# Stanford-ILIAD/Diverse-Conventions

Measured on NVIDIA B200. Metric: agent-steps/sec (env+obs), higher is better.
Workload: dtype u8

## Files before the change

### diverse_conventions_b200/csrc/policy_kernels.cu

```cuda
#include <cuda_bf16.h>
#include <cuda_runtime.h>
#include <stdint.h>
#include <stdlib.h>
#include <string.h>

#include <new>
#include <vector>

#include "api_common.h"
#include "oc_core.cuh"
#include "oc_device.cuh"
#include "mixed_schedule.h"
#include "ocb.h"
#include "policy_internal.h"

using namespace ocb;

namespace {

constexpr int kRows = 128;
constexpr int kHid = 64;
constexpr int kCo = 32;
constexpr int kSlots = 16;
constexpr int kK1 = 9 * kSlots;
// ... 406 lines not shown
    PB_COL_EMPTY = B_COL_EMPTY,
    PB_D1_FULL = 8,
    PB_A2_FULL = 10,
    PB_A2_EMPTY = 12,
    PB_D2_FULL = 14,
    PB_D3_FULL = 16,
    PB_D3_EMPTY = 18,
    PB_HEAD_FULL = 20,
    PB_HEAD_EMPTY = 21,
    PB_W_FULL = 24,
    PB_W_EMPTY = 48,
    PB_D1_EMPTY = 72,
    PBS_D1_FULL = 74,
    PBS_D1_EMPTY = 78,
    PB_COUNT = 82,
    PB_TMEM_SLOT = 120
};

struct PairSmemLayout {
    int stage, head, wring, bars, total;
};
__host__ __device__ inline PairSmemLayout pair_smem_layout(int npos, int ring, int stage_stride) {
    PairSmemLayout s;
    const BlobLayout L = blob_layout(npos);
    int o = 0;
    s.stage = o, o += al128(kLoadWarps * 32 * stage_stride * 4);
    s.head = o, o += kPRestOff + 2 * (L.head_bytes - L.bias1);
    s.wring = o, o += ring * kChunk;
    s.bars = o, o += 1024;
    s.total = o + 128;
    return s;
}

template <bool kProf, bool kPop = false, bool kMix = false>
__device__ __forceinline__ void pair_producer_role(long long* pw, const PolicyParams& prm, int t0, int t1, const BlobLayout L,
                                                   uint32_t s_head, uint32_t s_wring, uint32_t bars,
                                                   const uint8_t* mix_partner = nullptr) {
    const int nets = prm.single ? 1 : 2;
    const int R = prm.pair_ring, nch = nets * L.chunks;
    const bool resident = R >= nch;
    const bool static_w = resident && prm.tile_policy == nullptr;
    const int Reff = resident ? nch : R;
    const uint32_t rest = (uint32_t)(L.head_bytes - L.bias1);
    uint32_t u = 0, round = 0;
    int slot = 0;
    for (int t = t0; t < t1; ++t, ++u) {
        if (static_w && u > 0) break;
        const bool chg = blob_changed(prm, t, t0);
        const int tp = tile_pol(prm, t);
        const bool cross = prm.f_vt_round != 0 && prm.tile_policy != nullptr;
        const uint8_t* blob_a = prm.blobs + ((size_t)(cross ? (tp & 0xFFFF) : tp) * 2 + (prm.single == 2 ? 1 : 0)) * prm.blob_stride;
        const uint8_t* blob_c = kMix ? mix_partner
                                     : cross && !kPop ? prm.blobs + (size_t)(tp >> 16) * 2 * prm.blob_stride : blob_a + prm.blob_stride;
        if (chg) {
            if (u > 0) mbar_wait_p<kProf>(bars + 8 * (PB_HEAD_EMPTY + ((u - 1) & 1)), ((u - 1) >> 1) & 1, pw[PW_HEAD_EMPTY]);
            if (elect_one()) {
                const uint32_t hb = bars + 8 * PB_HEAD_FULL;
                mbar_arrive_expect_tx(hb, (uint32_t)nets * (2u * kPConvBytes + rest));
                bulk_g2s(s_head, blob_a + L.wc_hi, kPConvBytes, hb);
                bulk_g2s(s_head + 2 * kPConvBytes, blob_a + L.wc_lo, kPConvBytes, hb);
                bulk_g2s(s_head + kPRestOff, blob_a + L.bias1, rest, hb);
                if (nets == 2) {
                    bulk_g2s(s_head + kPConvBytes, blob_c + L.wc_hi, kPConvBytes, hb);
                    bulk_g2s(s_head + 3 * kPConvBytes, blob_c + L.wc_lo, kPConvBytes, hb);
                    bulk_g2s(s_head + kPRestOff + rest, blob_c + L.bias1, rest, hb);
                }
            }
            __syncwarp();
        }
        const bool load = !resident || chg;
        for (int j = 0; j < L.chunks; ++j) {
#pragma unroll
            for (int g = 0; g < 2; ++g) {
                if (g >= nets) break;
                if (round > 0) mbar_wait_p<kProf>(bars + 8 * (PB_W_EMPTY + slot), (round - 1) & 1, pw[PW_W_EMPTY]);
                if (load) {
                    if (elect_one()) {
                        mbar_arrive_expect_tx(bars + 8 * (PB_W_FULL + slot), kChunk);
                        bulk_g2s(s_wring + slot * kChunk, (g ? blob_c : blob_a) + L.head_bytes + (size_t)j * kChunk, kChunk,
                                 bars + 8 * (PB_W_FULL + slot));
                    }
                    __syncwarp();
                }
                if (++slot == Reff) slot = 0, ++round;
            }
        }
    }
}

template <bool kProf, int kNet>
__device__ __forceinline__ void pair_conv_role(long long* pw, const PolicyParams& prm, int t0, int t1, const BlobLayout L, uint32_t tmem,
                                               uint32_t a_head, uint32_t bars, const int cp0 = 0, const int cpstep = 1,
                                               const uint32_t ring = kColRing, const int col_full = PB_COL_FULL,
                                               const int col_empty = PB_COL_EMPTY) {
    const int W = prm.W, H = prm.H, PH = H - 2, npos = prm.npos;
    constexpr int kN = kNet < 0 ? kHid : kCo;
    const uint32_t idesc = make_idesc(kRows, kN);
    const uint32_t a_wchi = a_head + (kNet == 1 ? kPConvBytes : 0), a_wclo = a_wchi + 2 * kPConvBytes;
    const int b_full = kNet < 0 ? PB_D1_FULL : PBS_D1_FULL + 2 * kNet, b_empty = kNet < 0 ? PB_D1_EMPTY : PBS_D1_EMPTY + 2 * kNet;
    uint32_t head_gen = 0, u = 0;
    uint32_t uses[2] = {0, 0};
    const bool tracer = kNet <= 0;
    uint32_t t_slot = 0, t_round = 0;
    auto advance = [&](uint32_t& slot, uint32_t& round, int n) {
        for (int i = 0; i < n; ++i)
            if (++slot == ring) slot = 0, ++round;
    };

    for (int t = t0; t < t1; ++t, ++u) {
        if (blob_changed(prm, t, t0)) {
            mbar_wait_p<kProf>(bars + 8 * PB_HEAD_FULL, head_gen & 1, pw[PW_HEAD_FULL]);
            ++head_gen;
        }
        if (kNet == 1) {
            const int s_last = (npos - 1) & 1;
            const uint32_t cum = (u + 1) * (uint32_t)((npos + 1 - s_last) / 2);
            mbar_wait_p<kProf>(bars + 8 * (PBS_D1_FULL + s_last), (cum - 1) & 1, pw[PW_D3_FULL]);
        }
        uint32_t w_slot = t_slot, w_round = t_round;
        uint32_t r_slot = t_slot;
        uint32_t c_slot = t_slot;
        int cols_seen = 0, released = 0, ox = 0, oy = cp0;
        while (oy >= PH) oy -= PH, ++ox, c_slot = (c_slot + 1 == ring) ? 0 : c_slot + 1;
        for (int cp = cp0; cp < npos; cp += cpstep) {
            const int st = cp & 1;
            for (; cols_seen < ox + 3; ++cols_seen) {
                mbar_wait_p<kProf>(bars + 8 * (col_full + w_slot), w_round & 1, pw[PW_COL_FULL]);
                if (++w_slot == ring) w_slot = 0, ++w_round;
            }
            if (uses[st] > 0) mbar_wait_p<kProf>(bars + 8 * (b_empty + st), (uses[st] - 1) & 1, pw[PW_D1_FULL]);
            if (u > 0 && cp < 2 && !prm.single)
                mbar_wait_p<kProf>(bars + 8 * (PB_D3_EMPTY + (kNet < 0 ? cp : kNet)), (u - 1) & 1, pw[PW_D3_FULL]);
            tc_fence_after();
            const uint32_t d1 = tmem + kPColD1 + (kNet < 0 ? st * kHid : kNet * kHid + st * kCo);
            int nox = ox, noy = oy + cpstep;
            uint32_t n_slot = c_slot;
            while (noy >= PH) noy -= PH, ++nox, n_slot = (n_slot + 1 == ring) ? 0 : n_slot + 1;
            const int keep = cp + cpstep < npos ? nox : W;
            const uint32_t s1 = (c_slot + 1 >= ring) ? c_slot + 1 - ring : c_slot + 1;
            const uint32_t s2 = (c_slot + 2 >= ring) ? c_slot + 2 - ring : c_slot + 2;
            const uint32_t cellb = tmem + kColCells + (uint32_t)oy * kCellCols, colw = (uint32_t)H * kCellCols;
            const uint32_t cb0 = cellb + c_slot * colw, cb1 = cellb + s1 * colw, cb2 = cellb + s2 * colw;
            const long long ti0 = kProf ? clock64() : 0;
            if (cp == 3 && tracer) trace_ev<kProf>(prm, t - t0, 54);
            if (cp < 2 && tracer) trace_ev<kProf>(prm, t - t0, 11 + cp);
            if (elect_one()) {
#pragma unroll
                for (int j = 0; j < 9; ++j) {
                    const int dx = j / 3, dy = j - dx * 3;
                    const uint32_t ta = (dx == 0 ? cb0 : dx == 1 ? cb1 : cb2) + dy * kCellCols;
                    umma_bf16_ts(d1, ta, make_desc(a_wchi + j * 256, 128, 2304), idesc, j > 0);
                    umma_bf16_ts(d1, ta, make_desc(a_wclo + j * 256, 128, 2304), idesc, 1);
                }
                umma_commit(bars + 8 * (b_full + st));
                uint32_t rs = r_slot;
                for (int c = released; c < keep; ++c) {
                    umma_commit(bars + 8 * (col_empty + rs));
                    rs = (rs + 1 == ring) ? 0 : rs + 1;
                }
                if (cp + cpstep >= npos) umma_commit(bars + 8 * (PB_HEAD_EMPTY + (u & 1)));
            }
            __syncwarp();
            for (; released < keep; ++released) r_slot = (r_slot + 1 == ring) ? 0 : r_slot + 1;
            if (kProf) pw[PW_ISSUE_CONV] += clock64() - ti0;
            if (cp < 8 && tracer) trace_ev<kProf>(prm, t - t0, 16 + cp);
            ++uses[st];
            ox = nox, oy = noy, c_slot = n_slot;
        }
        advance(t_slot, t_round, W);
    }
}

template <bool kProf, bool kSplit>
__device__ __forceinline__ void pair_fc_role(long long* pw, const PolicyParams& prm, const int g, int t0, int t1, const BlobLayout L,
                                             uint32_t tmem, uint32_t a_wring, uint32_t bars) {
    const int npos = prm.npos;
    const int nets = prm.single ? 1 : 2;
    const int R = prm.pair_ring, nch = nets * L.chunks;
    const bool resident = R >= nch;
    const bool static_w = resident && prm.tile_policy == nullptr;
    const int Reff = resident ? nch : R;
    const uint32_t idesc = make_idesc(kRows, kHid);
    const uint32_t a_hi = tmem + kPColA2 + g * kA2Cols, a_lo = a_hi + 16;
    uint32_t item = 0, u = 0, w_gen = 0, wround = 0;
    int slot = g;
// ... 106 lines not shown
#pragma unroll 1
        for (int half = 0; half < 2; ++half) {
            float v[32];
            tmem_ld32(trow + kPColD2 + g * kHid + half * 32, v);
            publish(v, s_b1 + half * 32);
        }

        const uint32_t drawn = net == 0 ? out.draw(t, trow_id) : 0u;
        mbar_wait_p<kProf>(bars + 8 * (PB_D3_FULL + g), u & 1, pw[PW_D3_FULL]);
        if (kProf && (warp & 3) == 0) trace_ev<kProf>(prm, trace_vt, g == 0 ? 49 : 52);
        tc_fence_after();
        float head[6];
#pragma unroll
        for (int a = 0; a < 6; ++a) head[a] = s_bh[a];
#pragma unroll 1
        for (int half = 0; half < 2; ++half) {
            float v[32];
            tmem_ld32(trow + kPColD1 + g * kHid + half * 32, v);
            if (half == 1) {
                tc_fence_before();
                mbar_arrive(bars + 8 * (PB_D3_EMPTY + g));
            }
            head_accumulate(net, v, s_b2 + half * 32, s_wh, half * 32, head);
        }
        mbar_arrive(bars + 8 * (PB_HEAD_EMPTY + (u & 1)));
        if (kProf && (warp & 3) == 0) trace_ev<kProf>(prm, trace_vt, g == 0 ? 50 : 53);
        out(t, trow_id, net, head, drawn);
        if (kProf && warp == 0) trace_ev<kProf>(prm, trace_vt, 51);
    }
}
constexpr int kSColD3 = kPColD2 + kHid;
constexpr int kSHeadGroup = 1;

template <bool kProf>
__device__ __forceinline__ void single_fc_role(long long* pw, const PolicyParams& prm, int t0, int t1, const BlobLayout L, uint32_t tmem,
                                               uint32_t a_wring, uint32_t bars) {
    const int npos = prm.npos;
    const int R = prm.pair_ring, nch = L.chunks;
    const bool resident = R >= nch;
    const bool static_w = resident && prm.tile_policy == nullptr;
    const int Reff = resident ? nch : R;
    const uint32_t idesc = make_idesc(kRows, kHid);
    uint32_t u = 0, w_gen = 0, wround = 0;
    uint32_t cnt0 = 0, cnt1 = 0;
    int slot = 0;
    for (int t = t0; t < t1; ++t, ++u) {
        const bool chg = blob_changed(prm, t, t0);
        const bool w_loaded = !resident || chg;
        if (resident && w_loaded) ++w_gen;
        for (int j = 0; j < npos + 2; ++j) {
            const int sg = j < npos ? (j & 1) : (j - npos);
            const uint32_t k = sg ? cnt1 : cnt0;
            mbar_wait_p<kProf>(bars + 8 * (PB_A2_FULL + sg), k & 1, pw[PW_A2_FULL]);
            if (sg) ++cnt1; else ++cnt0;
            if (j == npos && u > 0) mbar_wait_p<kProf>(bars + 8 * PB_D3_EMPTY, (u - 1) & 1, pw[PW_D3_FULL]);
            if (w_loaded) mbar_wait_p<kProf>(bars + 8 * (PB_W_FULL + slot), resident ? ((w_gen - 1) & 1) : (wround & 1), pw[PW_W_FULL]);
            tc_fence_after();
            const uint32_t dst = tmem + (j < npos ? kPColD2 : kSColD3);
            const bool first = (j == 0 || j == npos);
            const uint32_t a_hi = tmem + kPColA2 + sg * kA2Cols, a_lo = a_hi + 16;
            const uint32_t b_hi = a_wring + slot * kChunk, b_lo = b_hi + 4096;
            const long long tf0 = kProf ? clock64() : 0;
            if (elect_one()) {
#pragma unroll
                for (int ks = 0; ks < 2; ++ks) {
                    const uint64_t bhi = make_desc(b_hi + ks * 256, 128, 512), blo = make_desc(b_lo + ks * 256, 128, 512);
                    umma_bf16_ts(dst, a_hi + ks * 8, bhi, idesc, (!first || ks != 0) ? 1u : 0u);
                    umma_bf16_ts(dst, a_hi + ks * 8, blo, idesc, 1);
                    umma_bf16_ts(dst, a_lo + ks * 8, bhi, idesc, 1);
                }
                umma_commit(bars + 8 * (PB_A2_EMPTY + sg));
                if (!static_w) umma_commit(bars + 8 * (PB_W_EMPTY + slot));
                if (j == npos - 1) umma_commit(bars + 8 * PB_D2_FULL);
                if (j == npos + 1) umma_commit(bars + 8 * PB_D3_FULL);
            }
            __syncwarp();
            if (kProf) pw[PW_ISSUE_FC] += clock64() - tf0;
            if (++slot >= Reff) slot = 0, ++wround;
        }
    }
}

template <bool kProf, class Out>
__device__ __forceinline__ void single_epilogue_role(long long* pw, const PolicyParams& prm, int t0, int t1, const BlobLayout L,
                                                     uint32_t tmem, const uint8_t* s_head, uint32_t bars, Out&& out) {
    const int warp = threadIdx.x >> 5, g = warp >> 2, trow_id = (warp & 3) * 32 + (threadIdx.x & 31);
    const int npos = prm.npos;
    const int net = prm.single == 2 ? 1 : 0;
    const uint32_t trow = tmem + ((uint32_t)((warp & 3) * 32) << 16);
    const uint8_t* rest = s_head + kPRestOff - L.bias1;
    const float* s_bias1 = reinterpret_cast<const float*>(rest + L.bias1);
    const float* s_b1 = reinterpret_cast<const float*>(rest + L.b1);
    const float* s_b2 = reinterpret_cast<const float*>(rest + L.b2);
    const float* s_wh = reinterpret_cast<const float*>(rest + L.wh);
    const float* s_bh = reinterpret_cast<const float*>(rest + L.bh);
    uint32_t u = 0, head_gen = 0, pubs = 0, d1_uses = 0;
    auto publish = [&](float (&v)[32], const float* bias) {
        const uint32_t a2 = trow + kPColA2 + g * kA2Cols;
        const float4* b4 = reinterpret_cast<const float4*>(bias);
        uint32_t hi[16], lo[16];
#pragma unroll
        for (int q = 0; q < 8; ++q) {
            const float4 b = b4[q];
            split2(fmaxf(v[4 * q] + b.x, 0.0f), fmaxf(v[4 * q + 1] + b.y, 0.0f), hi[2 * q], lo[2 * q]);
            split2(fmaxf(v[4 * q + 2] + b.z, 0.0f), fmaxf(v[4 * q + 3] + b.w, 0.0f), hi[2 * q + 1], lo[2 * q + 1]);
        }
        if (pubs >= 1) {
            mbar_wait_p<kProf>(bars + 8 * (PB_A2_EMPTY + g), (pubs - 1) & 1, pw[PW_A2_EMPTY]);
            tc_fence_after();
        }
        tmem_st16(a2, hi);
        tmem_st16(a2 + 16, lo);
        tmem_st_wait();
        tc_fence_before();
        mbar_arrive(bars + 8 * (PB_A2_FULL + g));
        ++pubs;
    };
    for (int t = t0; t < t1; ++t, ++u) {
        if (blob_changed(prm, t, t0)) {
            mbar_wait_p<kProf>(bars + 8 * PB_HEAD_FULL, head_gen & 1, pw[PW_HEAD_FULL]);
            ++head_gen;
        }
        for (int j = g; j < npos; j += 2, ++d1_uses) {
            mbar_wait_p<kProf>(bars + 8 * (PBS_D1_FULL + g), d1_uses & 1, pw[PW_D1_FULL]);
            tc_fence_after();
            float v[32];
            tmem_ld32(trow + kPColD1 + g * kCo, v);
            tc_fence_before();
            mbar_arrive(bars + 8 * (PBS_D1_EMPTY + g));
            publish(v, s_bias1 + j * kCo);
        }
        mbar_wait_p<kProf>(bars + 8 * PB_D2_FULL, u & 1, pw[PW_D2_FULL]);
        tc_fence_after();
        {
            float v[32];
            tmem_ld32(trow + kPColD2 + g * 32, v);
            publish(v, s_b1 + g * 32);
        }
        if (g != kSHeadGroup) {
            mbar_arrive(bars + 8 * (PB_HEAD_EMPTY + (u & 1)));
            continue;
        }
        const uint32_t drawn = net == 0 ? out.draw(t, trow_id) : 0u;
        mbar_wait_p<kProf>(bars + 8 * PB_D3_FULL, u & 1, pw[PW_D3_FULL]);
        tc_fence_after();
        float head[6];
#pragma unroll
        for (int a = 0; a < 6; ++a) head[a] = s_bh[a];
#pragma unroll 1
        for (int half = 0; half < 2; ++half) {
            float v[32];
            tmem_ld32(trow + kSColD3 + half * 32, v);
            if (half == 1) {
                tc_fence_before();
                mbar_arrive(bars + 8 * PB_D3_EMPTY);
            }
            head_accumulate(net, v, s_b2 + half * 32, s_wh, half * 32, head);
        }
        mbar_arrive(bars + 8 * (PB_HEAD_EMPTY + (u & 1)));
        out(t, trow_id, net, head, drawn);
    }
}

struct PairForwardOut {
    const PolicyParams& prm;
    unsigned long long offset;
    __device__ __forceinline__ PairForwardOut(const PolicyParams& p) : prm(p), offset(p.offset) {
        if (p.d_offset != nullptr) offset += *p.d_offset;
    }
    __device__ __forceinline__ uint32_t draw(int t, int trow_id) const {
        if (prm.deterministic || prm.given_actions != nullptr || !(prm.actions || prm.logp)) return 0u;
        return policy_draw(prm, (uint32_t)((long long)t * kRows + trow_id), offset);
    }
    __device__ __forceinline__ void operator()(int t, int trow_id, int net, const float (&head)[6], uint32_t drawn) const {
        const long long row = (long long)t * kRows + trow_id;
        if (row < prm.M) {
            if (net == 1) {
                if (prm.values) prm.values[row] = head[0];
            } else {
                emit_actor_row(prm, row, (uint32_t)row, head, offset, false, &drawn);
            }
        }
    }
};

template <bool kProf>
__global__ void __launch_bounds__(kPThreads, 1) policy_pair_kernel(const PolicyParams prm) {
    extern __shared__ uint8_t smem_raw[];
    uint8_t* smem = smem_raw + ((128u - (smem_addr(smem_raw) & 127u)) & 127u);
    const int tid = threadIdx.x, warp = tid >> 5;
// ... 199 lines not shown
        }
        p->pair_ring = ring;
        p->pair_smem_bytes = (size_t)pair_smem_layout(p->npos, ring, p->stage_stride).total;
    } else if (c5_smem_layout(p->npos, p->stage_stride).total > kSmemBudget + 128) {
        delete p;
        return fail(OCB_ERR_UNSUPPORTED, "layout too large for the hidden-512 conv kernel (%d x %d)", cfg->width, cfg->height);
    }
    DeviceGuard guard(device);
    const size_t bytes = generic ? 256 : (size_t)n_policies * 2 * (hidden == kHid ? (size_t)p->L.total : p->L5.total);
    cudaError_t err = cudaDeviceGetAttribute(&p->sm_count, cudaDevAttrMultiProcessorCount, device);
    if (err == cudaSuccess) err = cudaMalloc(&p->d_blobs, bytes);
    if (err == cudaSuccess) err = cudaMemset(p->d_blobs, 0, bytes);
    if (generic) {
        const size_t gbytes = (size_t)n_policies * 2 * p->LG.total * sizeof(float);
        if (err == cudaSuccess) err = cudaMalloc(&p->d_gblobs, gbytes);
        if (err == cudaSuccess) err = cudaMemset(p->d_gblobs, 0, gbytes);
        if (err == cudaSuccess) err = cudaFuncSetAttribute(policy_generic_kernel<kHid>, cudaFuncAttributeMaxDynamicSharedMemorySize, kSmemBudget + 128);
        if (err == cudaSuccess) err = cudaFuncSetAttribute(policy_generic_kernel<kH5>, cudaFuncAttributeMaxDynamicSharedMemorySize, kSmemBudget + 128);
    }
    const int smem_max = kSmemBudget + 128;
    if (err == cudaSuccess) err = cudaFuncSetAttribute(policy_pair_kernel<false>, cudaFuncAttributeMaxDynamicSharedMemorySize, smem_max);
    if (err == cudaSuccess) err = cudaFuncSetAttribute(policy_pair_kernel<true>, cudaFuncAttributeMaxDynamicSharedMemorySize, smem_max);
    if (err == cudaSuccess) err = cudaFuncSetAttribute(rollout_fused_kernel<false, false, 1>, cudaFuncAttributeMaxDynamicSharedMemorySize, smem_max);
    if (err == cudaSuccess) err = cudaFuncSetAttribute(rollout_fused_kernel<true, false, 1>, cudaFuncAttributeMaxDynamicSharedMemorySize, smem_max);
    if (err == cudaSuccess) err = cudaFuncSetAttribute(rollout_fused_kernel<false, true, 1>, cudaFuncAttributeMaxDynamicSharedMemorySize, smem_max);
    if (err == cudaSuccess) err = cudaFuncSetAttribute(rollout_fused_kernel<true, true, 1>, cudaFuncAttributeMaxDynamicSharedMemorySize, smem_max);
    if (err == cudaSuccess) err = cudaFuncSetAttribute(rollout_fused_kernel<false, false, 2>, cudaFuncAttributeMaxDynamicSharedMemorySize, smem_max);
    if (err == cudaSuccess) err = cudaFuncSetAttribute(rollout_fused_kernel<true, false, 2>, cudaFuncAttributeMaxDynamicSharedMemorySize, smem_max);
    if (err == cudaSuccess) err = cudaFuncSetAttribute(rollout_fused_kernel<false, false, 1, true>, cudaFuncAttributeMaxDynamicSharedMemorySize, smem_max);
    if (err == cudaSuccess) err = cudaFuncSetAttribute(rollout_fused_kernel<false, true, 1, true>, cudaFuncAttributeMaxDynamicSharedMemorySize, smem_max);
    if (err == cudaSuccess) err = cudaFuncSetAttribute(rollout_fused_kernel<false, false, 2, true>, cudaFuncAttributeMaxDynamicSharedMemorySize, smem_max);
    if (err == cudaSuccess) err = cudaFuncSetAttribute(rollout_fused_kernel<false, false, 1, false, true>, cudaFuncAttributeMaxDynamicSharedMemorySize, smem_max);
    if (err == cudaSuccess) err = cudaFuncSetAttribute(rollout_fused_kernel<false, false, 2, false, true>, cudaFuncAttributeMaxDynamicSharedMemorySize, smem_max);
    if (err == cudaSuccess) err = cudaFuncSetAttribute(conv512_kernel, cudaFuncAttributeMaxDynamicSharedMemorySize, smem_max);
    if (err == cudaSuccess) err = cudaFuncSetAttribute(gemm512_kernel<false, false>, cudaFuncAttributeMaxDynamicSharedMemorySize, smem_max);
    if (err == cudaSuccess) err = cudaFuncSetAttribute(gemm512_kernel<true, true>, cudaFuncAttributeMaxDynamicSharedMemorySize, smem_max);
    if (err != cudaSuccess) {
        cudaGetLastError();
        ocb_policy_destroy(p);
        return fail(OCB_ERR_CUDA, "ocb_policy_create: %s", cudaGetErrorString(err));
    }
    *out = p;
    return OCB_OK;
}

static int set_weights512(ocb_policy* p, int policy, int net, const float* conv_w, const float* conv_b, const float* fc1_w,
                          const float* fc1_b, const float* fc2_w, const float* fc2_b, const float* head_w, const float* head_b) {
    const Blob5& L = p->L5;
    std::vector<uint8_t> blob(L.total, 0);
    const int npos = p->npos, PH = p->H - 2;
    static const int slot_channel[kSlots] = {0, 1, 2, 3, 4, 5, 6, 7, 8, 9, 16, 17, 18, 19, 15, -1};
    for (int co = 0; co < kCo5; ++co)
        for (int j = 0; j < 9; ++j)
            for (int s = 0; s < kSlots; ++s) {
                const int ch = slot_channel[s];
                const float w = ch < 0 ? 0.0f : conv_w[((co * 20 + ch) * 3 + j / 3) * 3 + j % 3];
                put_split(blob.data() + L.wc_hi, blob.data() + L.wc_lo, canon_off(co, j * kSlots + s, kK1), w);
            }
    float* bias1 = reinterpret_cast<float*>(blob.data() + L.bias1);
    for (int pos = 0; pos < npos; ++pos) {
        const int ox = pos / PH, oy = pos % PH;
        for (int co = 0; co < kCo5; ++co) {
            double acc = conv_b[co];
            for (int dx = 0; dx < 3; ++dx)
                for (int dy = 0; dy < 3; ++dy) {
                    const int t = p->terrain[(oy + dy) * p->W + ox + dx];
// ... 369 lines not shown
    memset(&fp, 0, sizeof(fp));
    fp.pol.blobs = tile_policy != nullptr ? p->d_blobs : p->d_blobs + (size_t)policy_index * 2 * (size_t)p->L.total;
    fp.pol.blob_stride = (size_t)p->L.total;
    fp.pol.W = p->W, fp.pol.H = p->H, fp.pol.S = p->S, fp.pol.SC = p->SC, fp.pol.npos = p->npos;
    fp.pol.M = kRows, fp.pol.tiles = 1;
    fp.pol.deterministic = deterministic, fp.pol.seed = seed, fp.pol.offset = 0;
    fp.pol.rng_rows_per_seat = p->rng_rows_per_seat, fp.pol.rng_add0 = p->rng_add0, fp.pol.rng_add1 = p->rng_add1;
    fp.pol.d_offset = reinterpret_cast<const unsigned long long*>(d_offset);
    fp.pol.net_mask = 3, fp.pol.pair_ring = ring, fp.pol.stage_stride = p->stage_stride;
    fp.pol.tile_policy = tile_policy, fp.pol.f_vt_round = slots * (T + 1), fp.pol.f_slots = slots;
    fp.pol.f_seat1_tiles = population ? 0 : envp.N / kRows;
    fp.env = envp;
    fp.T = T, fp.wtiles = wtiles, fp.slots = slots, fp.cross = cross ? 1 : 0;
    fp.obs_slab = obs_slab, fp.actions = actions, fp.logp = logp, fp.values = values, fp.reward = reward, fp.done = done;
    if (mixed) {
        fp.mix_L = mix->L, fp.mix_seed = mix->mix_seed, fp.mix_partner_seed = mix->partner_seed;
        fp.mix_partner_blobs = p->d_blobs + (size_t)mix->partner_policy * 2 * (size_t)p->L.total;
    }
    const int groups = (wtiles + slots - 1) / slots;
    const int ctas = groups < p->sm_count ? groups : p->sm_count;
    const size_t smem = (size_t)fused_smem_layout(p->npos, ring, p->S, p->SC, slots).total;
    fp.pol.trace = d_trace, fp.pol.trace_u0 = trace_u0, fp.pol.trace_n = trace_n;
    {
        const char* e = getenv("OCB_FUSED_VEC_LOADER");
        fp.vec_loader = e != nullptr ? (e[0] != '0') : (p->SC % 16 == 0);
    }
    {
        const int cols = 192 / (kCellCols * p->H);
        const char* e = getenv("OCB_FUSED_SPLIT");
        const bool want = e != nullptr ? (e[0] != '0') : true;
        fp.col_ring = (want && slots == 1 && !cross && !mixed && cols >= p->W) ? (p->W < kFMaxColRing ? p->W : kFMaxColRing) : 0;
        if (fp.col_ring < p->W) fp.col_ring = 0;
    }
    const cudaStream_t st = (cudaStream_t)stream;
    if (mixed) {
        fp.col_ring = kColRing;
        if (slots == 2)
            rollout_fused_kernel<false, false, 2, false, true><<<ctas, kFThreads, smem, st>>>(fp);
        else
            rollout_fused_kernel<false, false, 1, false, true><<<ctas, kFThreads, smem, st>>>(fp);
    } else if (population) {
        if (fp.col_ring > 0) {
            rollout_fused_kernel<false, true, 1, true><<<ctas, kFThreads, smem, st>>>(fp);
        } else {
            fp.col_ring = kColRing;
            if (slots == 2)
                rollout_fused_kernel<false, false, 2, true><<<ctas, kFThreads, smem, st>>>(fp);
            else
                rollout_fused_kernel<false, false, 1, true><<<ctas, kFThreads, smem, st>>>(fp);
        }
    } else if (fp.col_ring > 0) {
        if (d_trace != nullptr)
            rollout_fused_kernel<true, true, 1><<<ctas, kFThreads, smem, st>>>(fp);
        else
            rollout_fused_kernel<false, true, 1><<<ctas, kFThreads, smem, st>>>(fp);
    } else {
        fp.col_ring = kColRing;
        if (slots == 2) {
            if (d_trace != nullptr)
                rollout_fused_kernel<true, false, 2><<<ctas, kFThreads, smem, st>>>(fp);
            else
                rollout_fused_kernel<false, false, 2><<<ctas, kFThreads, smem, st>>>(fp);
        } else {
            if (d_trace != nullptr)
                rollout_fused_kernel<true, false, 1><<<ctas, kFThreads, smem, st>>>(fp);
            else
                rollout_fused_kernel<false, false, 1><<<ctas, kFThreads, smem, st>>>(fp);
        }
    }
    if (d_counter != nullptr)
        counter_add_kernel<<<1, 1, 0, (cudaStream_t)stream>>>(reinterpret_cast<unsigned long long*>(d_counter), (unsigned long long)T);
    cudaError_t err = cudaGetLastError();
    if (err != cudaSuccess) return fail(OCB_ERR_CUDA, "fused rollout launch failed: %s", cudaGetErrorString(err));
    p->calls += 1;
    return OCB_OK;
}
```

### diverse_conventions_b200/csrc/rollout_fused.cuh

```cuda
#pragma once

struct FusedParams {
    PolicyParams pol;
    RolloutParams env;
    int T;
    int wtiles;
    int8_t* obs_slab;
    int32_t* actions;
    float* logp;
    float* values;
    int32_t* reward;
    int32_t* done;
    int vec_loader;
    int col_ring;
    int slots;
    int cross;
    int mix_L;
    unsigned long long mix_seed, mix_partner_seed;
    const uint8_t* mix_partner_blobs;
};

constexpr int kFEnvWarps = 2;
constexpr int kFWarpConvC = kPWarpProd + 1;
constexpr int kFWarpEnv = kFWarpConvC + 1;
// ... 26 lines not shown
    s.tmpl = o, o += (int)align16((size_t)SC);
    s.envw = o;
    s.view_stride = (int)align16((size_t)32 * SC);
    s.env_warp_bytes = 2 * s.view_stride + (int)align16((size_t)S * 32 * 2);
    s.slot_bytes = kFEnvWarps * s.env_warp_bytes;
    o += slots * s.slot_bytes;
    s.total = o + 128;
    return s;
}

struct FusedCursor {
    int kt0, u, s, T, wtiles, stride, slots;
    bool two;
    __device__ __forceinline__ FusedCursor(const FusedParams& fp)
        : kt0((int)blockIdx.x * fp.slots), u(0), s(0), T(fp.T), wtiles(fp.wtiles), stride((int)gridDim.x * fp.slots), slots(fp.slots) {
        two = slots == 2 && kt0 + 1 < wtiles;
    }
    __device__ __forceinline__ int kt() const { return kt0 + s; }
    __device__ __forceinline__ void next() {
        if (two && s == 0) {
            s = 1;
            return;
        }
        s = 0;
        if (++u > T) u = 0, kt0 += stride, two = slots == 2 && kt0 + 1 < wtiles;
    }
};
__host__ __device__ inline int fused_virtual_tiles(int wtiles, int slots, int grid, int cta, int T) {
    int n = 0;
    for (int kt0 = cta * slots; kt0 < wtiles; kt0 += grid * slots) n += ((slots == 2 && kt0 + 1 < wtiles) ? 2 : 1) * (T + 1);
    return n;
}

template <bool kProf, bool kSplit>
__device__ __forceinline__ void fused_loader_role(const FusedParams& fp, uint32_t nvt, uint32_t tmem, const uint8_t* s_env,
                                                  const FusedSmemLayout& sl, uint32_t bars) {
    const int lwarp = (threadIdx.x >> 5) - kEpiWarps, lg = lwarp >> 2, lw = lwarp & 3, lane = threadIdx.x & 31;
    const int W = fp.pol.W, H = fp.pol.H, seg = 5 * H;
    const uint32_t* myrow0 = reinterpret_cast<const uint32_t*>(s_env + (lw & 1) * sl.env_warp_bytes + (lw >> 1) * sl.view_stride +
                                                               lane * fp.pol.SC);
    const uint32_t* myrow = myrow0;
    const uint32_t tcells = tmem + ((uint32_t)(lw * 32) << 16) + kColCells;
    const uint32_t ncols = nvt * (uint32_t)W;
    uint32_t lt = 0;
    int lx = lg;
    bool fresh = true;
    FusedCursor cur(fp);
    uint32_t seen[2] = {0, 0};
    for (uint32_t gc = lg; gc < ncols; gc += 2) {
        if (fresh) {
            myrow = myrow0 + cur.s * (sl.slot_bytes >> 2);
            mbar_wait(bars + 8 * (FB_OBS_FULL + cur.s), (cur.s ? seen[1] : seen[0]) & 1);
            if (kProf && lwarp == 0) trace_ev<kProf>(fp.pol, (int)lt, 8);
        }
        const bool first_col = fresh;
        fresh = false;
        const uint32_t ring = kSplit ? (uint32_t)fp.col_ring : (uint32_t)kColRing;
        const int slot = gc % ring;
        if (gc >= ring) {
            mbar_wait(bars + 8 * ((kSplit ? FB_COL_EMPTY : PB_COL_EMPTY) + slot), ((gc / ring) - 1) & 1);
            tc_fence_after();
        }
        if (fp.vec_loader) {
            const uint32_t* colp = myrow + lx * seg;
            const int r = (int)((reinterpret_cast<uintptr_t>(colp) >> 2) & 3);
            const uint4* src4 = reinterpret_cast<const uint4*>(colp - r);
            constexpr int kMaxVec = (5 * kMaxH + 3 + 3) / 4;
            const int nvec = (seg + r + 3) >> 2;
            uint32_t c[4 * kMaxVec];
    #pragma unroll
            for (int i = 0; i < kMaxVec; ++i) {
                if (i < nvec) {
                    const uint4 q = src4[i];
                    c[4 * i] = q.x, c[4 * i + 1] = q.y, c[4 * i + 2] = q.z, c[4 * i + 3] = q.w;
                } else {
                    c[4 * i] = c[4 * i + 1] = c[4 * i + 2] = c[4 * i + 3] = 0u;
                }
            }
            auto word = [&](int k) -> uint32_t {
                const uint32_t a = (r & 1) ? c[k + 1] : c[k], b = (r & 1) ? c[k + 3] : c[k + 2];
                return (r & 2) ? b : a;
            };
    #pragma unroll
            for (int y = 0; y < kMaxH; ++y) {
                if (y < H) {
                    uint32_t w[5];
    #pragma unroll
                    for (int q = 0; q < 5; ++q) w[q] = word(y * 5 + q);
                    const uint4 c0 = make_uint4(bytes_bf16x2(w[0], pair_sel(0, 1)), bytes_bf16x2(w[0], pair_sel(2, 3)),
                                                bytes_bf16x2(w[1], pair_sel(0, 1)), bytes_bf16x2(w[1], pair_sel(2, 3)));
                    const uint4 c1 = make_uint4(bytes_bf16x2(w[2], pair_sel(0, 1)), bytes_bf16x2(w[4], pair_sel(0, 1)),
                                                bytes_bf16x2(w[4], pair_sel(2, 3)), bytes_bf16x2(w[3], pair_sel(3, 4)));
                    tmem_st8(tcells + (slot * H + y) * kCellCols, c0, c1);
                }
            }
        } else {
            const uint32_t* mine = myrow + lx * seg;
            for (int y = 0; y < H; ++y) {
                uint32_t w[5];
#pragma unroll
                for (int q = 0; q < 5; ++q) w[q] = mine[y * 5 + q];
                const uint4 c0 = make_uint4(bytes_bf16x2(w[0], pair_sel(0, 1)), bytes_bf16x2(w[0], pair_sel(2, 3)),
                                            bytes_bf16x2(w[1], pair_sel(0, 1)), bytes_bf16x2(w[1], pair_sel(2, 3)));
                const uint4 c1 = make_uint4(bytes_bf16x2(w[2], pair_sel(0, 1)), bytes_bf16x2(w[4], pair_sel(0, 1)),
                                            bytes_bf16x2(w[4], pair_sel(2, 3)), bytes_bf16x2(w[3], pair_sel(3, 4)));
                tmem_st8(tcells + (slot * H + y) * kCellCols, c0, c1);
            }
        }
        tmem_st_wait();
        tc_fence_before();
        mbar_arrive(bars + 8 * ((kSplit ? FB_COL_FULL : PB_COL_FULL) + slot));
        if (kProf && lwarp == 0 && first_col) trace_ev<kProf>(fp.pol, (int)lt, 9);
        if (kProf && lw == 0 && lx >= 1 && lx <= 4) trace_ev<kProf>(fp.pol, (int)lt, 3 + lx);
        lx += 2;
        if (lx >= W) {
            mbar_arrive(bars + 8 * (FB_OBS_EMPTY + cur.s));
            if (kProf && lwarp == 0) trace_ev<kProf>(fp.pol, (int)lt, 10);
            if (cur.s) ++seen[1]; else ++seen[0];
            cur.next();
            lx -= W, ++lt, fresh = true;
        }
    }
}

__device__ __forceinline__ void bulk_wait_read_1() { asm volatile("cp.async.bulk.wait_group.read 1;" ::: "memory"); }

template <int P>
struct FusedSlot {
    World<P> w;
    int cur_return, ep_add;
    long long ret_add;
    int n, nbytes;
    int j;
    bool valid, tma_ok, tma_pending;
    int8_t* obs_ptr;
    int32_t *rew_ptr, *done_ptr;
    uint32_t vts, acts;
};

template <bool kProf, int kSlots, bool kMix = false>
__device__ __forceinline__ void fused_env_role(const FusedParams& fp, uint8_t* s_env, const FusedSmemLayout& sl, const Tables& tb,
                                               const uint8_t* tmpl, const uint8_t* s_act, uint32_t bars) {
    constexpr int P = 2;
    const int ew = (threadIdx.x >> 5) - kFWarpEnv, lane = threadIdx.x & 31;
    const Consts c = load_consts(tb);
    const int SC = tb.SC, N = fp.env.N, T = fp.T;
    const int view_stride = sl.view_stride;
    const size_t PN = (size_t)P * N, obs_view_stride = (size_t)N * SC, obs_step_stride = PN * SC;
    const bool store_obs = fp.obs_slab != nullptr;
// ... 141 lines not shown
        }
        if constexpr (kSlots == 1) step_pre(tb, c, q.w, myobjs, 32, pre);
    };

    auto end_tile = [&](FusedSlot<P>& q, int slot) {
        if (q.valid) {
            fp.env.players[q.n] = player_pack(q.w.pos[0], q.w.orient[0], q.w.held[0]);
            fp.env.players[(size_t)N + q.n] = player_pack(q.w.pos[1], q.w.orient[1], q.w.held[1]);
            store_world_objs<1>(tb, c, fp.env, q.n, 0, objs_of(slot));
            fp.env.timestep[q.n] = q.w.timestep;
            fp.env.cur_return[q.n] = q.cur_return;
            if (q.ep_add) {
                fp.env.ret_sum[q.n] += q.ret_add;
                fp.env.episodes[q.n] += q.ep_add;
            }
        }
        __syncwarp();
    };

    for (int kt0 = (int)blockIdx.x * kSlots; kt0 < fp.wtiles; kt0 += (int)gridDim.x * kSlots) {
        const bool two = kSlots == 2 && kt0 + 1 < fp.wtiles;
        begin_tile(sa, 0, kt0);
        if (kSlots == 2 && two) begin_tile(sb, 1, kt0 + 1);
        for (int u = 0; u <= T; ++u) {
            step_tile(sa, 0, u, kSlots == 2 && two && sb.tma_pending);
            if (kSlots == 2 && two) step_tile(sb, 1, u, sa.tma_pending);
        }
        end_tile(sa, 0);
        if (kSlots == 2 && two) end_tile(sb, 1);
    }
    if ((sa.tma_pending || (kSlots == 2 && sb.tma_pending)) && (kMix || lane == 0)) bulk_wait_read_all();
}

template <bool kMix = false>
struct FusedOut {
    const FusedParams& fp;
    uint8_t* s_act;
    uint32_t bars;
    unsigned long long base;
    FusedCursor cur;
    int g;
    bool partner_row;
    __device__ __forceinline__ FusedOut(const FusedParams& f, uint8_t* sa, uint32_t b) : fp(f), s_act(sa), bars(b), cur(f) {
        base = f.pol.offset;
        if (f.pol.d_offset != nullptr) base += *f.pol.d_offset;
        g = (int)(threadIdx.x >> 7);
        partner_row = false;
    }
    __device__ __forceinline__ bool mine(int trow_id) const {
        if constexpr (kMix)
            return partner_row == (g == 1);
        else
            return !fp.cross || (trow_id >> 6) == g;
    }
    __device__ __forceinline__ bool mix_partner_plays(int trow_id) const {
        const int n = cur.kt() * kFWorlds + (trow_id & (kFWorlds - 1)), seat = trow_id >> 6;
        if (n >= fp.env.N || cur.u >= fp.T || mix_forced_main(fp.mix_L, cur.u, n % (fp.mix_L - 1))) return false;
        return mix_draw_partner(fp.mix_seed, (uint32_t)(seat * fp.env.N + n), base + (unsigned long long)cur.u);
    }
    __device__ __forceinline__ uint32_t draw(int, int trow_id) {
        if constexpr (kMix) partner_row = mix_partner_plays(trow_id);
        if (fp.pol.deterministic || cur.u >= fp.T || !mine(trow_id)) return 0u;
        const int wl = trow_id & (kFWorlds - 1), seat = trow_id >> 6;
        const long long row = (long long)seat * fp.env.N + (cur.kt() * kFWorlds + wl);
        if constexpr (kMix) {
            if (g == 1) {
                PolicyParams kp = fp.pol;
                kp.seed = fp.mix_partner_seed;
                return policy_draw(kp, (uint32_t)row, base + (unsigned long long)cur.u);
            }
        }
        return policy_draw(fp.pol, (uint32_t)row, base + (unsigned long long)cur.u);
    }
    __device__ __forceinline__ void operator()(int, int trow_id, int net, const float (&head)[6], uint32_t drawn) {
        const int N = fp.env.N, wl = trow_id & (kFWorlds - 1), seat = trow_id >> 6, u = cur.u;
        const int n = cur.kt() * kFWorlds + wl;
        const long long row = (long long)seat * N + n;
        const long long store = (long long)u * 2 * N + row;
        if (net == 1) {
            if (n < N && fp.values != nullptr) fp.values[store] = head[0];
        } else if (u < fp.T && mine(trow_id)) {
            PolicyParams op = fp.pol;
            const bool valid = n < N;
            bool rec = valid;
            long long at = store;
            if constexpr (kMix) {
                const int j = valid ? n % (fp.mix_L - 1) : 0;
                rec = valid && g == 0 && mix_forced_main(fp.mix_L, u, j);
                at = ((long long)mix_record_slot(fp.mix_L, u, j) * 2 + seat) * N + n;
            }
            op.actions = rec ? fp.actions : nullptr, op.logp = rec ? fp.logp : nullptr, op.logits = nullptr;
            emit_actor_row(op, at, (uint32_t)row, head, base + (unsigned long long)u, true, &drawn, s_act + cur.s * 128 + trow_id,
                           bars + 8 * (FB_ACT_FULL + cur.s));
        }
        cur.next();
    }
};

template <bool kProf, bool kSplit, int kSlots, bool kPop = false, bool kMix = false>
__global__ void __launch_bounds__(kFThreads, 1) rollout_fused_kernel(const FusedParams fp) {
    extern __shared__ uint8_t smem_raw[];
    uint8_t* smem = smem_raw + ((128u - (smem_addr(smem_raw) & 127u)) & 127u);
    const int tid = threadIdx.x, warp = tid >> 5;
    const PolicyParams& prm = fp.pol;
    const BlobLayout L = blob_layout(prm.npos);
    const FusedSmemLayout sl = fused_smem_layout(prm.npos, prm.pair_ring, prm.S, prm.SC, fp.slots);
    uint8_t* s_head = smem + sl.head;
    uint8_t* s_wring = smem + sl.wring;
    uint64_t* s_bars = reinterpret_cast<uint64_t*>(smem + sl.bars);
    uint32_t* s_tmem = reinterpret_cast<uint32_t*>(s_bars + PB_TMEM_SLOT);
    uint8_t* s_act = smem + sl.act;
    Tables* s_tables = reinterpret_cast<Tables*>(smem + sl.tables);
    uint8_t* s_tmpl = smem + sl.tmpl;
    uint8_t* s_env = smem + sl.envw;
    const uint32_t bars = smem_addr(s_bars);

    if (warp == 0) {
        asm volatile("tcgen05.alloc.cta_group::1.sync.aligned.shared::cta.b32 [%0], %1;" ::"r"(smem_addr(s_tmem)),
                     "r"((uint32_t)kTmemCols)
                     : "memory");
        asm volatile("tcgen05.relinquish_alloc_permit.cta_group::1.sync.aligned;" ::: "memory");
    }
    if (tid == 32) {
        for (int i = 0; i < FB_COUNT; ++i) {
            uint32_t count = 1;
            if ((i >= PB_COL_FULL && i < PB_COL_FULL + 4) || (i >= PB_A2_FULL && i < PB_A2_FULL + 2) ||
                (i >= PB_D3_EMPTY && i < PB_D3_EMPTY + 2))
                count = 128;
            if (i >= PB_COL_EMPTY && i < PB_COL_EMPTY + 4) count = 2;
            if (i >= PB_HEAD_EMPTY && i < PB_HEAD_EMPTY + 2) count = 32 * kEpiWarps + (kSplit ? 3 : 2);
            if (i >= PB_D1_EMPTY && i < PB_D1_EMPTY + 2) count = 32 * kEpiWarps;
            if (i >= PBS_D1_EMPTY && i < PBS_D1_EMPTY + 4) count = 128;
            if (i >= FB_COL_FULL && i < FB_COL_FULL + kFMaxColRing) count = 128;
            if (i >= FB_COL_EMPTY && i < FB_COL_EMPTY + kFMaxColRing) count = 3;
            if (i >= FB_OBS_FULL && i < FB_OBS_FULL + 2) count = 32 * kFEnvWarps;
            if (i >= FB_OBS_EMPTY && i < FB_OBS_EMPTY + 2) count = 32 * kLoadWarps;
            if (i >= FB_ACT_FULL && i < FB_ACT_FULL + 2) count = 128;
            mbar_init(bars + 8 * i, count);
        }
        asm volatile("fence.mbarrier_init.release.cluster;" ::: "memory");
    }
    {
        const uint32_t* src = reinterpret_cast<const uint32_t*>(fp.env.tables);
        uint32_t* dst = reinterpret_cast<uint32_t*>(s_tables);
        for (int i = tid; i < (int)(sizeof(Tables) / 4); i += kFThreads) dst[i] = src[i];
        for (int i = tid; i < prm.SC; i += kFThreads) s_tmpl[i] = fp.env.tmpl[i];
    }
    tc_fence_before();
    __syncthreads();
    tc_fence_after();
    const uint32_t tmem = *s_tmem;
    const int nvt = fused_virtual_tiles(fp.wtiles, fp.slots, (int)gridDim.x, (int)blockIdx.x, fp.T);

    long long pw[kProf ? PW_COUNT : 1] = {};
    if (warp < kEpiWarps) {
        pair_epilogue_role<kProf, kSplit, kPop, kMix>(pw, prm, 0, nvt, L, tmem, s_head, bars, FusedOut<kMix>(fp, s_act, bars));
    } else if (warp < kWarpMma) {
        fused_loader_role<kProf, kSplit>(fp, (uint32_t)nvt, tmem, s_env, sl, bars);
    } else if (warp == kWarpMma || warp == kWarpConv2) {
        const int half = warp == kWarpMma ? 0 : 1;
        if (kSplit)
            pair_conv_role<kProf, 0>(pw, prm, 0, nvt, L, tmem, smem_addr(s_head), bars, half, 2, (uint32_t)fp.col_ring, FB_COL_FULL,
                                     FB_COL_EMPTY);
        else
            pair_conv_role<kProf, -1>(pw, prm, 0, nvt, L, tmem, smem_addr(s_head), bars, half, 2);
    } else if (warp == kPWarpProd) {
        pair_producer_role<kProf, kPop, kMix>(pw, prm, 0, nvt, L, smem_addr(s_head), smem_addr(s_wring), bars,
                                              kMix ? fp.mix_partner_blobs : nullptr);
    } else if (warp < kPWarpProd) {
        pair_fc_role<kProf, kSplit>(pw, prm, warp - kWarpFc, 0, nvt, L, tmem, smem_addr(s_wring), bars);
    } else if (warp == kFWarpConvC) {
        if (kSplit)
            pair_conv_role<kProf, 1>(pw, prm, 0, nvt, L, tmem, smem_addr(s_head), bars, 0, 1, (uint32_t)fp.col_ring, FB_COL_FULL,
                                     FB_COL_EMPTY);
    } else {
        fused_env_role<kProf, kSlots, kMix>(fp, s_env, sl, *s_tables, s_tmpl, s_act, bars);
    }
    __syncwarp();
    tc_fence_before();
    __syncthreads();
    if (warp == 0)
        asm volatile("tcgen05.dealloc.cta_group::1.sync.aligned.b32 %0, %1;" ::"r"(tmem), "r"((uint32_t)kTmemCols) : "memory");
}

__global__ void counter_add_kernel(unsigned long long* ctr, unsigned long long k) { *ctr += k; }
```

Measured before the change: 16.05 billion.

## Add seat-tiled fused rollout path for cross-play with two slots

Adds a kSeat variant of the fused rollout kernel for cross-play with two slots. Each tile now holds one seat's rows from two world slots, and the seat alternates per tile, so one network runs on 128 rows instead of splitting each tile across two nets at 64 rows apiece. The producer loads both heads and streams the FC weights of the current seat's net. The conv, epilogue, loader and output indexing are reworked to pick seat-specific weights and map slots. The path is on by default via an env var. It gives up weight residency and adds complexity in barrier and slot indexing.

Result: no change. 16.09 billion, median of 6 (+0.2%).

```diff
diff --git a/diverse_conventions_b200/csrc/policy_kernels.cu b/diverse_conventions_b200/csrc/policy_kernels.cu
--- a/diverse_conventions_b200/csrc/policy_kernels.cu
+++ b/diverse_conventions_b200/csrc/policy_kernels.cu
@@ -462,13 +462,14 @@
     return s;
 }
 
-template <bool kProf, bool kPop = false, bool kMix = false>
+template <bool kProf, bool kPop = false, bool kMix = false, bool kSeat = false>
 __device__ __forceinline__ void pair_producer_role(long long* pw, const PolicyParams& prm, int t0, int t1, const BlobLayout L,
                                                    uint32_t s_head, uint32_t s_wring, uint32_t bars,
                                                    const uint8_t* mix_partner = nullptr) {
     const int nets = prm.single ? 1 : 2;
+    const int head_nets = kSeat ? 2 : nets;
     const int R = prm.pair_ring, nch = nets * L.chunks;
-    const bool resident = R >= nch;
+    const bool resident = !kSeat && R >= nch;
     const bool static_w = resident && prm.tile_policy == nullptr;
     const int Reff = resident ? nch : R;
     const uint32_t rest = (uint32_t)(L.head_bytes - L.bias1);
@@ -486,11 +487,11 @@
             if (u > 0) mbar_wait_p<kProf>(bars + 8 * (PB_HEAD_EMPTY + ((u - 1) & 1)), ((u - 1) >> 1) & 1, pw[PW_HEAD_EMPTY]);
             if (elect_one()) {
                 const uint32_t hb = bars + 8 * PB_HEAD_FULL;
-                mbar_arrive_expect_tx(hb, (uint32_t)nets * (2u * kPConvBytes + rest));
+                mbar_arrive_expect_tx(hb, (uint32_t)head_nets * (2u * kPConvBytes + rest));
                 bulk_g2s(s_head, blob_a + L.wc_hi, kPConvBytes, hb);
                 bulk_g2s(s_head + 2 * kPConvBytes, blob_a + L.wc_lo, kPConvBytes, hb);
                 bulk_g2s(s_head + kPRestOff, blob_a + L.bias1, rest, hb);
-                if (nets == 2) {
+                if (head_nets == 2) {
                     bulk_g2s(s_head + kPConvBytes, blob_c + L.wc_hi, kPConvBytes, hb);
                     bulk_g2s(s_head + 3 * kPConvBytes, blob_c + L.wc_lo, kPConvBytes, hb);
                     bulk_g2s(s_head + kPRestOff + rest, blob_c + L.bias1, rest, hb);
@@ -499,6 +500,7 @@
             __syncwarp();
         }
         const bool load = !resident || chg;
+        const uint8_t* blob_s = kSeat && (u & 1) ? blob_c : blob_a;
         for (int j = 0; j < L.chunks; ++j) {
 #pragma unroll
             for (int g = 0; g < 2; ++g) {
@@ -507,7 +509,7 @@
                 if (load) {
                     if (elect_one()) {
                         mbar_arrive_expect_tx(bars + 8 * (PB_W_FULL + slot), kChunk);
-                        bulk_g2s(s_wring + slot * kChunk, (g ? blob_c : blob_a) + L.head_bytes + (size_t)j * kChunk, kChunk,
+                        bulk_g2s(s_wring + slot * kChunk, (g ? blob_c : blob_s) + L.head_bytes + (size_t)j * kChunk, kChunk,
                                  bars + 8 * (PB_W_FULL + slot));
                     }
                     __syncwarp();
@@ -518,7 +520,7 @@
     }
 }
 
-template <bool kProf, int kNet>
+template <bool kProf, int kNet, bool kSeat = false>
 __device__ __forceinline__ void pair_conv_role(long long* pw, const PolicyParams& prm, int t0, int t1, const BlobLayout L, uint32_t tmem,
                                                uint32_t a_head, uint32_t bars, const int cp0 = 0, const int cpstep = 1,
                                                const uint32_t ring = kColRing, const int col_full = PB_COL_FULL,
@@ -571,6 +573,7 @@
             const uint32_t s2 = (c_slot + 2 >= ring) ? c_slot + 2 - ring : c_slot + 2;
             const uint32_t cellb = tmem + kColCells + (uint32_t)oy * kCellCols, colw = (uint32_t)H * kCellCols;
             const uint32_t cb0 = cellb + c_slot * colw, cb1 = cellb + s1 * colw, cb2 = cellb + s2 * colw;
+            const uint32_t wseat = kSeat ? (u & 1) * kPConvBytes : 0;
             const long long ti0 = kProf ? clock64() : 0;
             if (cp == 3 && tracer) trace_ev<kProf>(prm, t - t0, 54);
             if (cp < 2 && tracer) trace_ev<kProf>(prm, t - t0, 11 + cp);
@@ -579,8 +582,8 @@
                 for (int j = 0; j < 9; ++j) {
                     const int dx = j / 3, dy = j - dx * 3;
                     const uint32_t ta = (dx == 0 ? cb0 : dx == 1 ? cb1 : cb2) + dy * kCellCols;
-                    umma_bf16_ts(d1, ta, make_desc(a_wchi + j * 256, 128, 2304), idesc, j > 0);
-                    umma_bf16_ts(d1, ta, make_desc(a_wclo + j * 256, 128, 2304), idesc, 1);
+                    umma_bf16_ts(d1, ta, make_desc(a_wchi + wseat + j * 256, 128, 2304), idesc, j > 0);
+                    umma_bf16_ts(d1, ta, make_desc(a_wclo + wseat + j * 256, 128, 2304), idesc, 1);
                 }
                 umma_commit(bars + 8 * (b_full + st));
                 uint32_t rs = r_slot;
@@ -753,12 +756,12 @@
 constexpr int kSColD3 = kPColD2 + kHid;
 constexpr int kSHeadGroup = 1;
 
-template <bool kProf>
+template <bool kProf, bool kSeat = false>
 __device__ __forceinline__ void single_fc_role(long long* pw, const PolicyParams& prm, int t0, int t1, const BlobLayout L, uint32_t tmem,
                                                uint32_t a_wring, uint32_t bars) {
     const int npos = prm.npos;
     const int R = prm.pair_ring, nch = L.chunks;
-    const bool resident = R >= nch;
+    const bool resident = !kSeat && R >= nch;
     const bool static_w = resident && prm.tile_policy == nullptr;
     const int Reff = resident ? nch : R;
     const uint32_t idesc = make_idesc(kRows, kHid);
@@ -802,7 +805,7 @@
     }
 }
 
-template <bool kProf, class Out>
+template <bool kProf, bool kSeat = false, class Out>
 __device__ __forceinline__ void single_epilogue_role(long long* pw, const PolicyParams& prm, int t0, int t1, const BlobLayout L,
                                                      uint32_t tmem, const uint8_t* s_head, uint32_t bars, Out&& out) {
     const int warp = threadIdx.x >> 5, g = warp >> 2, trow_id = (warp & 3) * 32 + (threadIdx.x & 31);
@@ -842,6 +845,7 @@
             mbar_wait_p<kProf>(bars + 8 * PB_HEAD_FULL, head_gen & 1, pw[PW_HEAD_FULL]);
             ++head_gen;
         }
+        const int hs = kSeat ? (int)(u & 1) * ((L.head_bytes - L.bias1) >> 2) : 0;
         for (int j = g; j < npos; j += 2, ++d1_uses) {
             mbar_wait_p<kProf>(bars + 8 * (PBS_D1_FULL + g), d1_uses & 1, pw[PW_D1_FULL]);
             tc_fence_after();
@@ -849,14 +853,14 @@
             tmem_ld32(trow + kPColD1 + g * kCo, v);
             tc_fence_before();
             mbar_arrive(bars + 8 * (PBS_D1_EMPTY + g));
-            publish(v, s_bias1 + j * kCo);
+            publish(v, s_bias1 + hs + j * kCo);
         }
         mbar_wait_p<kProf>(bars + 8 * PB_D2_FULL, u & 1, pw[PW_D2_FULL]);
         tc_fence_after();
         {
             float v[32];
             tmem_ld32(trow + kPColD2 + g * 32, v);
-            publish(v, s_b1 + g * 32);
+            publish(v, s_b1 + hs + g * 32);
         }
         if (g != kSHeadGroup) {
             mbar_arrive(bars + 8 * (PB_HEAD_EMPTY + (u & 1)));
@@ -867,7 +871,7 @@
         tc_fence_after();
         float head[6];
 #pragma unroll
-        for (int a = 0; a < 6; ++a) head[a] = s_bh[a];
+        for (int a = 0; a < 6; ++a) head[a] = s_bh[hs + a];
 #pragma unroll 1
         for (int half = 0; half < 2; ++half) {
             float v[32];
@@ -876,7 +880,7 @@
                 tc_fence_before();
                 mbar_arrive(bars + 8 * PB_D3_EMPTY);
             }
-            head_accumulate(net, v, s_b2 + half * 32, s_wh, half * 32, head);
+            head_accumulate(net, v, s_b2 + hs + half * 32, s_wh + hs, half * 32, head);
         }
         mbar_arrive(bars + 8 * (PB_HEAD_EMPTY + (u & 1)));
         out(t, trow_id, net, head, drawn);
@@ -1142,6 +1146,7 @@
     if (err == cudaSuccess) err = cudaFuncSetAttribute(rollout_fused_kernel<false, false, 2, true>, cudaFuncAttributeMaxDynamicSharedMemorySize, smem_max);
     if (err == cudaSuccess) err = cudaFuncSetAttribute(rollout_fused_kernel<false, false, 1, false, true>, cudaFuncAttributeMaxDynamicSharedMemorySize, smem_max);
     if (err == cudaSuccess) err = cudaFuncSetAttribute(rollout_fused_kernel<false, false, 2, false, true>, cudaFuncAttributeMaxDynamicSharedMemorySize, smem_max);
+    if (err == cudaSuccess) err = cudaFuncSetAttribute(rollout_fused_kernel<false, false, 2, false, false, true>, cudaFuncAttributeMaxDynamicSharedMemorySize, smem_max);
     if (err == cudaSuccess) err = cudaFuncSetAttribute(conv512_kernel, cudaFuncAttributeMaxDynamicSharedMemorySize, smem_max);
     if (err == cudaSuccess) err = cudaFuncSetAttribute(gemm512_kernel<false, false>, cudaFuncAttributeMaxDynamicSharedMemorySize, smem_max);
     if (err == cudaSuccess) err = cudaFuncSetAttribute(gemm512_kernel<true, true>, cudaFuncAttributeMaxDynamicSharedMemorySize, smem_max);
@@ -1577,6 +1582,11 @@
         fp.col_ring = (want && slots == 1 && !cross && !mixed && cols >= p->W) ? (p->W < kFMaxColRing ? p->W : kFMaxColRing) : 0;
         if (fp.col_ring < p->W) fp.col_ring = 0;
     }
+    bool seat_tiles = false;
+    if (cross && slots == 2) {
+        const char* e = getenv("OCB_FUSED_SEAT_TILES");
+        seat_tiles = e == nullptr || e[0] != '0';
+    }
     const cudaStream_t st = (cudaStream_t)stream;
     if (mixed) {
         fp.col_ring = kColRing;
@@ -1594,6 +1604,10 @@
             else
                 rollout_fused_kernel<false, false, 1, true><<<ctas, kFThreads, smem, st>>>(fp);
         }
+    } else if (seat_tiles) {
+        fp.col_ring = kColRing;
+        fp.pol.single = 1;
+        rollout_fused_kernel<false, false, 2, false, false, true><<<ctas, kFThreads, smem, st>>>(fp);
     } else if (fp.col_ring > 0) {
         if (d_trace != nullptr)
             rollout_fused_kernel<true, true, 1><<<ctas, kFThreads, smem, st>>>(fp);
diff --git a/diverse_conventions_b200/csrc/rollout_fused.cuh b/diverse_conventions_b200/csrc/rollout_fused.cuh
--- a/diverse_conventions_b200/csrc/rollout_fused.cuh
+++ b/diverse_conventions_b200/csrc/rollout_fused.cuh
@@ -82,13 +82,13 @@
     return n;
 }
 
-template <bool kProf, bool kSplit>
+template <bool kProf, bool kSplit, bool kSeat = false>
 __device__ __forceinline__ void fused_loader_role(const FusedParams& fp, uint32_t nvt, uint32_t tmem, const uint8_t* s_env,
                                                   const FusedSmemLayout& sl, uint32_t bars) {
     const int lwarp = (threadIdx.x >> 5) - kEpiWarps, lg = lwarp >> 2, lw = lwarp & 3, lane = threadIdx.x & 31;
     const int W = fp.pol.W, H = fp.pol.H, seg = 5 * H;
-    const uint32_t* myrow0 = reinterpret_cast<const uint32_t*>(s_env + (lw & 1) * sl.env_warp_bytes + (lw >> 1) * sl.view_stride +
-                                                               lane * fp.pol.SC);
+    const uint32_t* myrow0 = reinterpret_cast<const uint32_t*>(
+        s_env + (lw & 1) * sl.env_warp_bytes + (lw >> 1) * (kSeat ? sl.slot_bytes : sl.view_stride) + lane * fp.pol.SC);
     const uint32_t* myrow = myrow0;
     const uint32_t tcells = tmem + ((uint32_t)(lw * 32) << 16) + kColCells;
     const uint32_t ncols = nvt * (uint32_t)W;
@@ -99,8 +99,13 @@
     uint32_t seen[2] = {0, 0};
     for (uint32_t gc = lg; gc < ncols; gc += 2) {
         if (fresh) {
-            myrow = myrow0 + cur.s * (sl.slot_bytes >> 2);
-            mbar_wait(bars + 8 * (FB_OBS_FULL + cur.s), (cur.s ? seen[1] : seen[0]) & 1);
+            if constexpr (kSeat) {
+                myrow = myrow0 + cur.s * (sl.view_stride >> 2);
+                mbar_wait(bars + 8 * (FB_OBS_FULL + (lw >> 1)), (lt >> 1) & 1);
+            } else {
+                myrow = myrow0 + cur.s * (sl.slot_bytes >> 2);
+                mbar_wait(bars + 8 * (FB_OBS_FULL + cur.s), (cur.s ? seen[1] : seen[0]) & 1);
+            }
             if (kProf && lwarp == 0) trace_ev<kProf>(fp.pol, (int)lt, 8);
         }
         const bool first_col = fresh;
@@ -164,7 +169,7 @@
         if (kProf && lw == 0 && lx >= 1 && lx <= 4) trace_ev<kProf>(fp.pol, (int)lt, 3 + lx);
         lx += 2;
         if (lx >= W) {
-            mbar_arrive(bars + 8 * (FB_OBS_EMPTY + cur.s));
+            mbar_arrive(bars + 8 * (FB_OBS_EMPTY + (kSeat ? lw >> 1 : cur.s)));
             if (kProf && lwarp == 0) trace_ev<kProf>(fp.pol, (int)lt, 10);
             if (cur.s) ++seen[1]; else ++seen[0];
             cur.next();
@@ -372,7 +377,7 @@
     if ((sa.tma_pending || (kSlots == 2 && sb.tma_pending)) && (kMix || lane == 0)) bulk_wait_read_all();
 }
 
-template <bool kMix = false>
+template <bool kMix = false, bool kSeat = false>
 struct FusedOut {
     const FusedParams& fp;
     uint8_t* s_act;
@@ -388,7 +393,9 @@
         partner_row = false;
     }
     __device__ __forceinline__ bool mine(int trow_id) const {
-        if constexpr (kMix)
+        if constexpr (kSeat)
+            return true;
+        else if constexpr (kMix)
             return partner_row == (g == 1);
         else
             return !fp.cross || (trow_id >> 6) == g;
@@ -401,8 +408,9 @@
     __device__ __forceinline__ uint32_t draw(int, int trow_id) {
         if constexpr (kMix) partner_row = mix_partner_plays(trow_id);
         if (fp.pol.deterministic || cur.u >= fp.T || !mine(trow_id)) return 0u;
-        const int wl = trow_id & (kFWorlds - 1), seat = trow_id >> 6;
-        const long long row = (long long)seat * fp.env.N + (cur.kt() * kFWorlds + wl);
+        const int wl = trow_id & (kFWorlds - 1), seat = kSeat ? cur.s : trow_id >> 6;
+        const int kt = kSeat ? cur.kt0 + (trow_id >> 6) : cur.kt();
+        const long long row = (long long)seat * fp.env.N + (kt * kFWorlds + wl);
         if constexpr (kMix) {
             if (g == 1) {
                 PolicyParams kp = fp.pol;
@@ -413,8 +421,9 @@
         return policy_draw(fp.pol, (uint32_t)row, base + (unsigned long long)cur.u);
     }
     __device__ __forceinline__ void operator()(int, int trow_id, int net, const float (&head)[6], uint32_t drawn) {
-        const int N = fp.env.N, wl = trow_id & (kFWorlds - 1), seat = trow_id >> 6, u = cur.u;
-        const int n = cur.kt() * kFWorlds + wl;
+        const int N = fp.env.N, wl = trow_id & (kFWorlds - 1), seat = kSeat ? cur.s : trow_id >> 6, u = cur.u;
+        const int slot = kSeat ? trow_id >> 6 : cur.s;
+        const int n = (kSeat ? cur.kt0 + slot : cur.kt()) * kFWorlds + wl;
         const long long row = (long long)seat * N + n;
         const long long store = (long long)u * 2 * N + row;
         if (net == 1) {
@@ -430,14 +439,15 @@
                 at = ((long long)mix_record_slot(fp.mix_L, u, j) * 2 + seat) * N + n;
             }
             op.actions = rec ? fp.actions : nullptr, op.logp = rec ? fp.logp : nullptr, op.logits = nullptr;
-            emit_actor_row(op, at, (uint32_t)row, head, base + (unsigned long long)u, true, &drawn, s_act + cur.s * 128 + trow_id,
-                           bars + 8 * (FB_ACT_FULL + cur.s));
+            emit_actor_row(op, at, (uint32_t)row, head, base + (unsigned long long)u, true, &drawn,
+                           s_act + (kSeat ? slot * 128 + seat * kFWorlds + wl : cur.s * 128 + trow_id),
+                           bars + 8 * (FB_ACT_FULL + slot));
         }
         cur.next();
     }
 };
 
-template <bool kProf, bool kSplit, int kSlots, bool kPop = false, bool kMix = false>
+template <bool kProf, bool kSplit, int kSlots, bool kPop = false, bool kMix = false, bool kSeat = false>
 __global__ void __launch_bounds__(kFThreads, 1) rollout_fused_kernel(const FusedParams fp) {
     extern __shared__ uint8_t smem_raw[];
     uint8_t* smem = smem_raw + ((128u - (smem_addr(smem_raw) & 127u)) & 127u);
@@ -494,21 +504,30 @@
 
     long long pw[kProf ? PW_COUNT : 1] = {};
     if (warp < kEpiWarps) {
-        pair_epilogue_role<kProf, kSplit, kPop, kMix>(pw, prm, 0, nvt, L, tmem, s_head, bars, FusedOut<kMix>(fp, s_act, bars));
+        if constexpr (kSeat)
+            single_epilogue_role<kProf, true>(pw, prm, 0, nvt, L, tmem, s_head, bars, FusedOut<false, true>(fp, s_act, bars));
+        else
+            pair_epilogue_role<kProf, kSplit, kPop, kMix>(pw, prm, 0, nvt, L, tmem, s_head, bars, FusedOut<kMix>(fp, s_act, bars));
     } else if (warp < kWarpMma) {
-        fused_loader_role<kProf, kSplit>(fp, (uint32_t)nvt, tmem, s_env, sl, bars);
+        fused_loader_role<kProf, kSplit, kSeat>(fp, (uint32_t)nvt, tmem, s_env, sl, bars);
     } else if (warp == kWarpMma || warp == kWarpConv2) {
         const int half = warp == kWarpMma ? 0 : 1;
         if (kSplit)
             pair_conv_role<kProf, 0>(pw, prm, 0, nvt, L, tmem, smem_addr(s_head), bars, half, 2, (uint32_t)fp.col_ring, FB_COL_FULL,
                                      FB_COL_EMPTY);
+        else if (kSeat)
+            pair_conv_role<kProf, 0, true>(pw, prm, 0, nvt, L, tmem, smem_addr(s_head), bars, half, 2);
         else
             pair_conv_role<kProf, -1>(pw, prm, 0, nvt, L, tmem, smem_addr(s_head), bars, half, 2);
     } else if (warp == kPWarpProd) {
-        pair_producer_role<kProf, kPop, kMix>(pw, prm, 0, nvt, L, smem_addr(s_head), smem_addr(s_wring), bars,
-                                              kMix ? fp.mix_partner_blobs : nullptr);
+        pair_producer_role<kProf, kPop, kMix, kSeat>(pw, prm, 0, nvt, L, smem_addr(s_head), smem_addr(s_wring), bars,
+                                                     kMix ? fp.mix_partner_blobs : nullptr);
     } else if (warp < kPWarpProd) {
-        pair_fc_role<kProf, kSplit>(pw, prm, warp - kWarpFc, 0, nvt, L, tmem, smem_addr(s_wring), bars);
+        if constexpr (kSeat) {
+            if (warp == kWarpFc) single_fc_role<kProf, true>(pw, prm, 0, nvt, L, tmem, smem_addr(s_wring), bars);
+        } else {
+            pair_fc_role<kProf, kSplit>(pw, prm, warp - kWarpFc, 0, nvt, L, tmem, smem_addr(s_wring), bars);
+        }
     } else if (warp == kFWarpConvC) {
         if (kSplit)
             pair_conv_role<kProf, 1>(pw, prm, 0, nvt, L, tmem, smem_addr(s_head), bars, 0, 1, (uint32_t)fp.col_ring, FB_COL_FULL,
```
